# microsoft/ptgnn

Measured on NVIDIA H100. Metric: edges/sec per GNN layer, higher is better.
Workload: dtype f32

## Files before the change

ptgnn_b200/csrc/fused_mp.cu:

```cuda
#include "fused_mp.cuh"

#include <cuda_bf16.h>
#include <cuda_fp16.h>
#include <float.h>
#include <stdlib.h>

#include <type_traits>

#include "tc_common.cuh"

namespace ptgnn {
namespace fused {

using tc::mbar_arrive;
using tc::mbar_init;
using tc::mbar_wait;

constexpr int NUM_THREADS = 16 * 32;
constexpr int GATHER_WARP0 = 8, GATHER_THREADS = 64;
constexpr int SCHED_WARP = 10;
constexpr int REDUCER_WARP0 = 12;
constexpr int SCHED_READER_WARPS = 8 + 2 + 4;
constexpr int NUM_SLOTS = 3, LOOKAHEAD = 2;
constexpr int SLOT_BYTES = 32768;
constexpr int RING_BYTES = NUM_SLOTS * SLOT_BYTES;
constexpr int META_RING = 8;
constexpr int SCHED_RING = 4;
constexpr int PRODUCER_REGS = 56, CONSUMER_REGS = 184, REDUCER_REGS = 88;
static_assert(PRODUCER_REGS + 2 * CONSUMER_REGS + REDUCER_REGS <= 4 * 128, "register budgets exceed the launch allocation");
constexpr int NMAX = 64;
constexpr int ACC_PITCH = NMAX + 4;
constexpr int ACC_BYTES = kD * ACC_PITCH * 4;
constexpr int RED_BAR_ID = 1;

struct Meta {
    int32_t tloff[128];
    uint32_t endmask[4];
    int32_t n, pad[3];
};
struct Sched {
    int32_t blk, pad[3];
    int32_t off[PTGNN_MAX_EDGE_TYPES + 4];
};
constexpr int ACC_OFF = RING_BYTES;
constexpr int AGG_OFF = RING_BYTES + ACC_BYTES;
__host__ __device__ constexpr int agg_bytes(int B) { return B * kD * 4; }
constexpr int SMEM_TAIL = META_RING * (int)sizeof(Meta) + SCHED_RING * (int)sizeof(Sched) + 256 ;
constexpr int smem_bytes(int B) { return 1024 + RING_BYTES + ACC_BYTES + agg_bytes(B) + SMEM_TAIL; }
static_assert(smem_bytes(kMaxBlockTargets) <= 232448, "shared memory budget");

struct Params {
    const unsigned char *src_rows, *tgt_rows;
    const uint4 *wpack;
    const int32_t *group_off, *src_f;
    const uint8_t *tl_f;
    const int32_t *row_ptr;
    void *out;
    int num_nodes, num_blocks, B, T, reduce, out_mode;
    int32_t *status;
    unsigned long long *trace;
    Epilogue epi;
    EgcEpilogue egc;
};
constexpr int EPI_AGG = 0, EPI_EGC = 1;

__device__ __forceinline__ uint4 ldg_nc_u4(const uint4 *p) {
    uint4 r;
    asm volatile("ld.global.nc.L1::no_allocate.v4.u32 {%0,%1,%2,%3}, [%4];" : "=r"(r.x), "=r"(r.y), "=r"(r.z), "=r"(r.w) : "l"(p));
    return r;
}
__device__ __forceinline__ void named_bar_sync(int id, int threads) { asm volatile("bar.sync %0, %1;" ::"r"(id), "r"(threads) : "memory"); }
__device__ __forceinline__ uint32_t swz(int row, int q) { return (uint32_t)(row * 128 + ((q ^ (row & 7)) << 4)); }

constexpr int TRACE_ROLES = 4, TRACE_CAP = 8192;
__shared__ uint32_t trace_n[TRACE_ROLES];
__device__ __forceinline__ void trace_mark(const Params &p, int tag, uint32_t step) {
    if (p.trace == nullptr || blockIdx.x != 0) return;
    const int tid = (int)threadIdx.x;
    const int role = tid == GATHER_WARP0 * 32 ? 0 : (tid == 0 ? 1 : (tid == 128 ? 2 : (tid == REDUCER_WARP0 * 32 ? 3 : -1)));
    if (role < 0) return;
    const uint32_t n = trace_n[role];
    if (n >= TRACE_CAP) return;
    p.trace[role * TRACE_CAP + n] = ((unsigned long long)clock64() << 24) | ((unsigned long long)(step & 0xFFFFu) << 8) | (unsigned)(tag & 0xFF);
    trace_n[role] = n + 1;
}

struct Step { int blk, t, e, n, seg; };
template <int NSEG>
struct StepGen {
    const Sched *sched;
    uint64_t *sfull, *sempty;
    int T, nmax, lane;
    uint32_t it = 0;
    const Sched *tab = nullptr;
    int blk = -1, t = 0, e = 0, e1 = 0, seg = 0;
    __device__ __forceinline__ int next(Step &s) {
        for (;;) {
            if (tab == nullptr) {
                const uint32_t r = it % SCHED_RING;
                mbar_wait(&sfull[r], (it / SCHED_RING) & 1);
                blk = sched[r].blk;
                if (blk < 0) return 2;
                tab = &sched[r];
                t = -1; e = e1 = 0; seg = 0;
            }
            if (e < e1) {
                s.blk = blk; s.t = t; s.e = e; s.n = min(nmax, e1 - e); s.seg = seg;
                if (++seg == NSEG) { seg = 0; e += nmax; }
                return 0;
            }
            ++t;
            while (t < T && tab->off[t + 1] == tab->off[t]) ++t;
            if (t >= T) {
                tab = nullptr;
                s.blk = blk;
                __syncwarp();
                if (lane == 0) mbar_arrive(&sempty[it % SCHED_RING]);
                ++it;
                return 1;
            }
            e = tab->off[t]; e1 = tab->off[t + 1]; seg = 0;
        }
    }
};

template <int RED>
__device__ __forceinline__ void continue_segment(float &t, float prev, float v, uint32_t start_bit) {
    if (RED == PTGNN_REDUCE_MAX)
        asm("{\n\t.reg .pred pc;\n\tsetp.eq.u32 pc, %3, 0;\n\t@pc max.f32 %0, %1, %2;\n\t}" : "+f"(t) : "f"(prev), "f"(v), "r"(start_bit));
    else if (RED == PTGNN_REDUCE_MIN)
        asm("{\n\t.reg .pred pc;\n\tsetp.eq.u32 pc, %3, 0;\n\t@pc min.f32 %0, %1, %2;\n\t}" : "+f"(t) : "f"(prev), "f"(v), "r"(start_bit));
    else
        asm("{\n\t.reg .pred pc;\n\tsetp.eq.u32 pc, %3, 0;\n\t@pc add.f32 %0, %1, %2;\n\t}" : "+f"(t) : "f"(prev), "f"(v), "r"(start_bit));
}
__device__ __forceinline__ void sts_f32_if(uint32_t addr, float v, uint32_t bit) {
    asm volatile("{\n\t.reg .pred pe;\n\tsetp.ne.u32 pe, %2, 0;\n\t@pe st.shared.f32 [%0], %1;\n\t}" ::"r"(addr), "f"(v), "r"(bit) : "memory");
}
__device__ __forceinline__ float4 lds_f32x4(uint32_t addr) {
    float4 v;
    asm volatile("ld.shared.v4.f32 {%0, %1, %2, %3}, [%4];" : "=f"(v.x), "=f"(v.y), "=f"(v.z), "=f"(v.w) : "r"(addr));
    return v;
}
__device__ __forceinline__ void sts_f32x4(uint32_t addr, float4 v) {
    asm volatile("st.shared.v4.f32 [%0], {%1, %2, %3, %4};" ::"r"(addr), "f"(v.x), "f"(v.y), "f"(v.z), "f"(v.w) : "memory");
}
__device__ __forceinline__ float lds_f32(uint32_t addr) {
    float v;
    asm volatile("ld.shared.f32 %0, [%1];" : "=f"(v) : "r"(addr) : "memory");
    return v;
}

__device__ __forceinline__ uint32_t pack_h2(__half a, __half b) {
    return (uint32_t)__half_as_ushort(a) | ((uint32_t)__half_as_ushort(b) << 16);
}
__device__ __forceinline__ bool split_f16(float x, __half &hi, __half &lo) {
    hi = __float2half_rn(x);
    lo = __float2half_rn((x - __half2float(hi)) * 2048.0f);
    return fabsf(x) < 65504.0f;
}

template <int RED> __device__ __forceinline__ float red_identity() {
    return RED == PTGNN_REDUCE_MAX ? -FLT_MAX : (RED == PTGNN_REDUCE_MIN ? FLT_MAX : 0.0f);
}
template <int RED> __device__ __forceinline__ float red_op(float a, float m) {
    if (RED == PTGNN_REDUCE_MAX) return fmaxf(a, m);
    if (RED == PTGNN_REDUCE_MIN) return fminf(a, m);
    return a + m;
}

template <int RED>
__device__ __forceinline__ void write_out_block(const Params *p, uint32_t agg_saddr, int row0, int r_first, int r_step, int q) {
    const float IDENT = red_identity<RED>();
    const int my_hi = min(p->B, p->num_nodes - row0);
    const float4 ident4 = make_float4(IDENT, IDENT, IDENT, IDENT);
    auto finish_row = [&](auto mode_tag, auto plain_tag, int r, float4 a) {
        constexpr int MODE = decltype(mode_tag)::value;
        constexpr bool PLAIN = decltype(plain_tag)::value;
        const int v = row0 + r;
        if (!PLAIN) {
            if (RED == PTGNN_REDUCE_MEAN) {
                const int cnt = __ldg(p->row_ptr + v + 1) - __ldg(p->row_ptr + v);
                const float c = (float)(cnt < 1 ? 1 : cnt);
                a.x /= c; a.y /= c; a.z /= c; a.w /= c;
            }
            if (RED == PTGNN_REDUCE_MAX || RED == PTGNN_REDUCE_MIN) {
                if (a.x == IDENT) a.x = 0.0f;
                if (a.y == IDENT) a.y = 0.0f;
                if (a.z == IDENT) a.z = 0.0f;
                if (a.w == IDENT) a.w = 0.0f;
            }
            if (p->epi.act != PTGNN_ACT_NONE) {
                a.x = apply_act(a.x, p->epi.act); a.y = apply_act(a.y, p->epi.act);
                a.z = apply_act(a.z, p->epi.act); a.w = apply_act(a.w, p->epi.act);
            }
            if (p->epi.ln_w != nullptr) {
                float sum = (a.x + a.y) + (a.z + a.w);
#pragma unroll
                for (int o = 16; o > 0; o >>= 1) sum += __shfl_xor_sync(0xffffffffu, sum, o);
                const float mean = sum / (float)kD;
                const float dx = a.x - mean, dy = a.y - mean, dz = a.z - mean, dw = a.w - mean;
                float qq = (dx * dx + dy * dy) + (dz * dz + dw * dw);
#pragma unroll
                for (int o = 16; o > 0; o >>= 1) qq += __shfl_xor_sync(0xffffffffu, qq, o);
                const float rstd = rsqrtf(qq / (float)kD + p->epi.ln_eps);
                const float4 w = *reinterpret_cast<const float4 *>(p->epi.ln_w + q * 4);
                const float4 b = *reinterpret_cast<const float4 *>(p->epi.ln_b + q * 4);
                a.x = dx * rstd * w.x + b.x; a.y = dy * rstd * w.y + b.y;
                a.z = dz * rstd * w.z + b.z; a.w = dw * rstd * w.w + b.w;
            }
        }
        if (MODE == 1) {
            __nv_bfloat162 lo = __floats2bfloat162_rn(a.x, a.y), hi = __floats2bfloat162_rn(a.z, a.w);
            uint2 pk;
            pk.x = *reinterpret_cast<uint32_t *>(&lo); pk.y = *reinterpret_cast<uint32_t *>(&hi);
            reinterpret_cast<uint2 *>(p->out)[(size_t)v * (kD / 4) + q] = pk;
        } else if (MODE == 2) {
            const __half2 h01 = __floats2half2_rn(a.x, a.y), h23 = __floats2half2_rn(a.z, a.w);
            const float2 f01 = __half22float2(h01), f23 = __half22float2(h23);
            const __half2 l01 = __floats2half2_rn((a.x - f01.x) * 2048.0f, (a.y - f01.y) * 2048.0f);
            const __half2 l23 = __floats2half2_rn((a.z - f23.x) * 2048.0f, (a.w - f23.y) * 2048.0f);
            uint2 *row = reinterpret_cast<uint2 *>(p->out) + (size_t)v * (2 * kD / 4);
            row[q] = make_uint2(*reinterpret_cast<const uint32_t *>(&h01), *reinterpret_cast<const uint32_t *>(&h23));
            row[kD / 4 + q] = make_uint2(*reinterpret_cast<const uint32_t *>(&l01), *reinterpret_cast<const uint32_t *>(&l23));
            const float big = fmaxf(fmaxf(fabsf(a.x), fabsf(a.y)), fmaxf(fabsf(a.z), fabsf(a.w)));
            if (!(big < 65504.0f) && p->status != nullptr) *reinterpret_cast<volatile int32_t *>(p->status) = 1;
        } else {
            reinterpret_cast<float4 *>(p->out)[(size_t)v * (kD / 4) + q] = a;
        }
    };
    auto write_rows = [&](auto mode_tag, auto plain_tag) {
        for (int r0 = r_first; r0 < my_hi; r0 += 2 * r_step) {
            float4 v4[2];
#pragma unroll
            for (int u = 0; u < 2; ++u) {
                const int r = r0 + r_step * u;
                if (r < my_hi) {
                    const uint32_t rowa = agg_saddr + (uint32_t)(r * kD + q * 4) * 4u;
                    v4[u] = lds_f32x4(rowa);
                    sts_f32x4(rowa, ident4);
                }
            }
#pragma unroll
            for (int u = 0; u < 2; ++u)
                if (r0 + r_step * u < my_hi) finish_row(mode_tag, plain_tag, r0 + r_step * u, v4[u]);
        }
    };
    const bool plain = RED == PTGNN_REDUCE_SUM && p->epi.act == PTGNN_ACT_NONE && p->epi.ln_w == nullptr;
    using std::integral_constant;
    if (p->out_mode == 2) { if (plain) write_rows(integral_constant<int, 2>{}, integral_constant<bool, true>{}); else write_rows(integral_constant<int, 2>{}, integral_constant<bool, false>{}); }
    else if (p->out_mode == 1) { if (plain) write_rows(integral_constant<int, 1>{}, integral_constant<bool, true>{}); else write_rows(integral_constant<int, 1>{}, integral_constant<bool, false>{}); }
    else { if (plain) write_rows(integral_constant<int, 0>{}, integral_constant<bool, true>{}); else write_rows(integral_constant<int, 0>{}, integral_constant<bool, false>{}); }
}

__device__ __forceinline__ float bf16r(float x) { return __bfloat162float(__float2bfloat16_rn(x)); }

template <int RED>
__device__ __forceinline__ void write_out_block_egc(const Params *p, uint32_t agg_saddr, int row0, int r_first, int r_step, int q) {
    const float IDENT = red_identity<RED>();
    const int my_hi = min(p->B, p->num_nodes - row0);
    const float4 ident4 = make_float4(IDENT, IDENT, IDENT, IDENT);
    const EgcEpilogue &e = p->egc;
    const bool bf = p->out_mode == 1;
    for (int r = r_first; r < my_hi; r += r_step) {
        const uint32_t rowa = agg_saddr + (uint32_t)(r * kD + q * 4) * 4u;
        const float4 a4 = lds_f32x4(rowa);
        sts_f32x4(rowa, ident4);
        const int v = row0 + r;
        float x[4] = {a4.x, a4.y, a4.z, a4.w};
        float cdiv = 1.0f;
        if (RED == PTGNN_REDUCE_MEAN) {
            const int cnt = __ldg(p->row_ptr + v + 1) - __ldg(p->row_ptr + v);
            cdiv = (float)(cnt < 1 ? 1 : cnt);
        }
#pragma unroll
        for (int i = 0; i < 4; ++i) {
            if (RED == PTGNN_REDUCE_MEAN) x[i] /= cdiv;
            if ((RED == PTGNN_REDUCE_MAX || RED == PTGNN_REDUCE_MIN) && x[i] == IDENT) x[i] = 0.0f;
            if (bf) x[i] = bf16r(x[i]);
        }
        const float *crow = e.coef + (size_t)v * e.coef_stride;
        auto prod = [&](float A, float w) { const float t = __fmul_rn(A, w); return bf ? bf16r(t) : t; };
        const size_t orow = (size_t)v * e.out_stride;
        auto store1 = [&](int o, float s) {
            if (bf) reinterpret_cast<__nv_bfloat16 *>(p->out)[orow + o] = __float2bfloat16_rn(s);
            else reinterpret_cast<float *>(p->out)[orow + o] = s;
        };
        if (e.bases == 4 || e.bases == 8) {
            const int o = e.col0 + (e.bases == 4 ? q : q >> 1);
            const int b0 = e.bases == 4 ? 0 : 4 * (q & 1);
            const float4 w = *reinterpret_cast<const float4 *>(crow + (o / e.dh) * e.bases + b0);
            const float p0 = prod(x[0], w.x), p1 = prod(x[1], w.y), p2 = prod(x[2], w.z), p3 = prod(x[3], w.w);
            float s = __fadd_rn(__fadd_rn(__fadd_rn(p0, p1), p2), p3);
            if (e.bases == 8) {
                const float lower = __shfl_xor_sync(0xffffffffu, s, 1);
                s = __fadd_rn(__fadd_rn(__fadd_rn(__fadd_rn(lower, p0), p1), p2), p3);
                if ((q & 1) == 0) continue;
            }
            store1(o, s);
        } else if (e.bases == 2) {
            const int o = e.col0 + 2 * q;
            const float2 w0 = *reinterpret_cast<const float2 *>(crow + (o / e.dh) * 2);
            const float2 w1 = *reinterpret_cast<const float2 *>(crow + ((o + 1) / e.dh) * 2);
            const float s0 = __fadd_rn(prod(x[0], w0.x), prod(x[1], w0.y));
            const float s1 = __fadd_rn(prod(x[2], w1.x), prod(x[3], w1.y));
            if (bf) *reinterpret_cast<__nv_bfloat162 *>(reinterpret_cast<__nv_bfloat16 *>(p->out) + orow + o) = __floats2bfloat162_rn(s0, s1);
            else *reinterpret_cast<float2 *>(reinterpret_cast<float *>(p->out) + orow + o) = make_float2(s0, s1);
        } else {
            const int o = e.col0 + 4 * q;
            float s[4];
#pragma unroll
            for (int i = 0; i < 4; ++i) s[i] = prod(x[i], __ldg(crow + (o + i) / e.dh));
            if (bf) {
                __nv_bfloat162 lo = __floats2bfloat162_rn(s[0], s[1]), hi = __floats2bfloat162_rn(s[2], s[3]);
                uint2 pk;
                pk.x = *reinterpret_cast<uint32_t *>(&lo); pk.y = *reinterpret_cast<uint32_t *>(&hi);
                *reinterpret_cast<uint2 *>(reinterpret_cast<__nv_bfloat16 *>(p->out) + orow + o) = pk;
            } else {
                *reinterpret_cast<float4 *>(reinterpret_cast<float *>(p->out) + orow + o) = make_float4(s[0], s[1], s[2], s[3]);
            }
        }
    }
}

template <int NPROD, int K, int NSEG, int RED, int EPI>
__global__ void __launch_bounds__(NUM_THREADS, 1) fused_aggregate_kernel(const __grid_constant__ Params p) {
    constexpr int NPART = NPROD == 3 ? 2 : 1;
    constexpr int ROW_BYTES = K * 2 * NPART;
    constexpr int KCH = K / 64;
    constexpr int NT = NPART * KCH;
    constexpr int TILE_BYTES = NMAX * 128;
    static_assert(NT * TILE_BYTES <= SLOT_BYTES, "slot size");
    constexpr bool BF16 = NPROD == 1;

    extern __shared__ unsigned char smem_raw[];
    unsigned char *ring = smem_raw + ((1024u - (smem_u32(smem_raw) & 1023u)) & 1023u);
    float *acc_s = reinterpret_cast<float *>(ring + ACC_OFF);
    float *agg_s = reinterpret_cast<float *>(ring + AGG_OFF);
    unsigned char *tail = ring + AGG_OFF + agg_bytes(p.B);
    Meta *meta_ring = reinterpret_cast<Meta *>(tail);
    Sched *sched = reinterpret_cast<Sched *>(tail + META_RING * sizeof(Meta));
    uint64_t *bars = reinterpret_cast<uint64_t *>(tail + META_RING * sizeof(Meta) + SCHED_RING * sizeof(Sched));
    uint64_t *x_full = bars, *x_empty = bars + 3, *sched_full = bars + 6, *sched_empty = bars + 10;
    uint64_t *acc_full = bars + 14, *acc_empty = bars + 15;

    const int warp = __shfl_sync(0xffffffffu, (int)(threadIdx.x >> 5), 0);
    const int lane = threadIdx.x & 31;
    if (threadIdx.x == 0) {
        for (int s = 0; s < NUM_SLOTS; ++s) { mbar_init(&x_full[s], 2 * GATHER_THREADS); mbar_init(&x_empty[s], 8); }
        for (int r = 0; r < SCHED_RING; ++r) { mbar_init(&sched_full[r], 1); mbar_init(&sched_empty[r], SCHED_READER_WARPS); }
        mbar_init(acc_full, 8);
        mbar_init(acc_empty, 4);
        for (int r = 0; r < TRACE_ROLES; ++r) trace_n[r] = 0;
        tc::mbar_init_fence();
    }
    __syncthreads();
    const int T = p.T;

    if (warp >= REDUCER_WARP0) {
        tc::reg_dealloc<REDUCER_REGS>();
        const int d = (int)threadIdx.x - REDUCER_WARP0 * 32, rw = warp - REDUCER_WARP0;
        const uint32_t aggcol_s = smem_u32(agg_s + d);
        const uint32_t accrow_s = smem_u32(acc_s + d * ACC_PITCH);
        const float IDENT = red_identity<RED>();
        for (int r = 0; r < p.B; ++r) agg_s[r * kD + d] = IDENT;
        StepGen<NSEG> gen{sched, sched_full, sched_empty, T, NMAX, lane};
        uint32_t sg = 0;
        float acc = IDENT;
        Step s;
        for (int ev; (ev = gen.next(s)) != 2;) {
            if (ev == 1) {
                trace_mark(p, 33, sg);
                named_bar_sync(RED_BAR_ID, 128);
                if constexpr (EPI == EPI_EGC) write_out_block_egc<RED>(&p, smem_u32(agg_s), s.blk * p.B, rw, 4, lane);
                else write_out_block<RED>(&p, smem_u32(agg_s), s.blk * p.B, rw, 4, lane);
                named_bar_sync(RED_BAR_ID, 128);
                trace_mark(p, 34, sg);
                continue;
            }
            if (s.seg != NSEG - 1) continue;
            trace_mark(p, 30, sg);
            mbar_wait(acc_full, sg & 1);
            trace_mark(p, 31, sg);
            const Meta *m = &meta_ring[sg % META_RING];
            const int n = s.n;
            constexpr int W = 16;
            for (int c0 = 0; c0 < n; c0 += W) {
                uint32_t vm[W];
#pragma unroll
                for (int j = 0; j < W / 4; ++j) {
                    const float4 v4 = lds_f32x4(accrow_s + (uint32_t)(c0 + 4 * j) * 4u);
                    vm[4 * j] = __float_as_uint(v4.x); vm[4 * j + 1] = __float_as_uint(v4.y);
                    vm[4 * j + 2] = __float_as_uint(v4.z); vm[4 * j + 3] = __float_as_uint(v4.w);
                }
                uint32_t addr[W];
#pragma unroll
                for (int j = 0; j < W / 4; ++j) {
                    const int4 o = *reinterpret_cast<const int4 *>(&m->tloff[c0 + 4 * j]);
                    addr[4 * j] = aggcol_s + o.x; addr[4 * j + 1] = aggcol_s + o.y;
                    addr[4 * j + 2] = aggcol_s + o.z; addr[4 * j + 3] = aggcol_s + o.w;
                }
                const uint32_t endw = (m->endmask[c0 >> 5] >> (c0 & 31)) & 0xFFFFu;
                const uint32_t prev_end = c0 == 0 ? 1u : (m->endmask[(c0 - 1) >> 5] >> ((c0 - 1) & 31)) & 1u;
                const uint32_t startw = (endw << 1) | prev_end;
                float pre[W];
#pragma unroll
                for (int c = 0; c < W; ++c) pre[c] = lds_f32(addr[c]);
                float t[W];
                constexpr bool ADD = RED == PTGNN_REDUCE_SUM || RED == PTGNN_REDUCE_MEAN;
#pragma unroll
                for (int c = 0; c < W; ++c) {
                    const float v = __uint_as_float(vm[c]);
                    t[c] = ADD ? __fadd_rn(pre[c], v) : red_op<RED>(pre[c], v);
                }
                continue_segment<RED>(t[0], acc, __uint_as_float(vm[0]), startw & 1u);
#pragma unroll
                for (int c = 1; c < W; ++c) continue_segment<RED>(t[c], t[c - 1], __uint_as_float(vm[c]), startw & (1u << c));
                acc = t[W - 1];
#pragma unroll
                for (int c = 0; c < W; ++c) sts_f32_if(addr[c], t[c], endw & (1u << c));
            }
            __syncwarp();
            if (lane == 0) mbar_arrive(acc_empty);
            trace_mark(p, 32, sg);
            ++sg;
        }
    } else if (warp >= GATHER_WARP0) {
        tc::reg_dealloc<PRODUCER_REGS>();
        if (warp == SCHED_WARP) {
            for (uint32_t i = 0;; ++i) {
                const uint32_t r = i % SCHED_RING;
                mbar_wait(&sched_empty[r], ((i / SCHED_RING) & 1) ^ 1);
                const long long blk = (long long)blockIdx.x + (long long)i * gridDim.x;
                const bool valid = blk < p.num_blocks;
                Sched *e = &sched[r];
                if (valid) {
                    for (int t = lane; t <= T; t += 32) e->off[t] = __ldg(p.group_off + blk * T + t);
                }
                if (lane == 0) e->blk = valid ? (int)blk : -1;
                __syncwarp();
                if (lane == 0) mbar_arrive(&sched_full[r]);
                if (!valid) break;
            }
        } else if (warp < GATHER_WARP0 + GATHER_THREADS / 32) {
            const int g = (int)threadIdx.x - GATHER_WARP0 * 32;
            const int q = g & 7, rsub = g >> 3;
            StepGen<NSEG> gen{sched, sched_full, sched_empty, T, NMAX, lane};
            uint32_t c_issue = 0, c_done = 0, sgc = 0;
            Step cur, nxt;
            bool has_nxt = false;
            int idx_nxt[NMAX / 8];
            int tl_a[NMAX / 64], tl_b[NMAX / 64];
            auto fetch = [&]() {
                int ev;
                do { ev = gen.next(nxt); } while (ev == 1);
                has_nxt = ev == 0;
                if (!has_nxt) return;
                if (nxt.seg == 0) {
#pragma unroll
                    for (int i = 0; i < NMAX / 8; ++i) {
                        const int r = rsub + 8 * i;
                        idx_nxt[i] = r < nxt.n ? __ldg(p.src_f + nxt.e + r) : -1;
                    }
#pragma unroll
                    for (int half = 0; half < NMAX / 64; ++half) {
                        const int c = g + 64 * half;
                        tl_a[half] = c < nxt.n ? (int)__ldg(p.tl_f + nxt.e + c) : -1;
                        tl_b[half] = c + 1 < nxt.n ? (int)__ldg(p.tl_f + nxt.e + c + 1) : -2;
                    }
                } else {
#pragma unroll
                    for (int i = 0; i < NMAX / 8; ++i) {
                        const int r = rsub + 8 * i;
                        idx_nxt[i] = r < nxt.n ? nxt.blk * p.B + (int)__ldg(p.tl_f + nxt.e + r) : -1;
                    }
                }
            };
            auto finish_meta = [&](const Step &st) {
                if (st.seg != 0) return;
                Meta *m = &meta_ring[sgc % META_RING];
#pragma unroll
                for (int half = 0; half < NMAX / 64; ++half) {
                    const int c = g + 64 * half;
                    const bool valid = tl_a[half] >= 0;
                    const bool end = valid && tl_b[half] != tl_a[half];
                    m->tloff[c] = valid ? tl_a[half] * (kD * 4) : 0;
                    const uint32_t word = __ballot_sync(0xffffffffu, end);
                    if (lane == 0) m->endmask[c >> 5] = word;
                }
                if (g == 0) m->n = st.n;
                ++sgc;
            };
            auto issue_next = [&]() {
                cur = nxt;
                int idx[NMAX / 8];
#pragma unroll
                for (int i = 0; i < NMAX / 8; ++i) idx[i] = idx_nxt[i];
                finish_meta(cur);
                const uint32_t slot = c_issue % NUM_SLOTS;
                trace_mark(p, 1, c_issue);
                mbar_wait(&x_empty[slot], ((c_issue / NUM_SLOTS) & 1) ^ 1);
                trace_mark(p, 2, c_issue);
                const unsigned char *rows = cur.seg == 0 ? p.src_rows : p.tgt_rows;
                const uint32_t sbase = smem_u32(ring + slot * SLOT_BYTES) + swz(rsub, q);
#pragma unroll
                for (int i = 0; i < NMAX / 8; ++i) {
                    if (idx[i] >= 0) {
                        const unsigned char *src = rows + (size_t)idx[i] * ROW_BYTES + q * 16;
#pragma unroll
                        for (int ti = 0; ti < NT; ++ti)
                            cp_async16(sbase + ti * TILE_BYTES + i * 1024, src + (ti / KCH) * (K * 2) + (ti % KCH) * 128, 16);
                    }
                }
                trace_mark(p, 3, c_issue);
                ++c_issue;
            };
            fetch();
            bool more = has_nxt;
            while (more) {
                const uint32_t slot = c_issue % NUM_SLOTS;
                issue_next();
                asm volatile("cp.async.mbarrier.arrive.noinc.shared::cta.b64 [%0];" ::"r"(smem_u32(&x_full[slot])) : "memory");
                trace_mark(p, 4, c_done);
                mbar_arrive(&x_full[slot]);
                ++c_done;
                fetch();
                more = has_nxt;
            }
            cp_async_wait<0>();
        }
    } else {
        tc::reg_alloc<CONSUMER_REGS>();
        const int eg = warp >> 2, ew = warp & 3;
        const int gq = lane >> 2, tq = lane & 3;
        const int f0 = 64 * eg + 16 * ew + gq;
        StepGen<NSEG> gen{sched, sched_full, sched_empty, T, NMAX, lane};
        uint32_t sg = 0, xs = 0;
        int w_t = -1, w_seg = -1;
        uint32_t wf[NPART][K / 16][4];
        float acc_m[32], acc_c[32];
        auto load_weights = [&](const Step &st) {
            const uint32_t *wp = reinterpret_cast<const uint32_t *>(p.wpack + (size_t)(st.t * NSEG + st.seg) * NPART * (K / 8) * 128);
#pragma unroll
            for (int part = 0; part < NPART; ++part)
#pragma unroll
                for (int ks = 0; ks < K / 16; ++ks)
#pragma unroll
                    for (int i = 0; i < 4; ++i) {
                        const int c4 = (part * (K / 8) + 2 * ks + (i >> 1)), f = f0 + 8 * (i & 1);
                        wf[part][ks][i] = __ldg(wp + ((size_t)c4 * 128 + f) * 4 + tq);
                    }
            w_t = st.t; w_seg = st.seg;
            trace_mark(p, 11, xs);
        };
        auto mma = [&](auto nb_tag, uint32_t slot_addr) {
            constexpr int NB = decltype(nb_tag)::value;
#pragma unroll
            for (int ks = 0; ks < K / 16; ++ks) {
                const int kc = ks >> 2, kk = ks & 3;
                const uint64_t x_hi = tc::make_smem_desc_sw128(slot_addr + kc * TILE_BYTES) + kk * 2;
                const uint64_t x_lo = tc::make_smem_desc_sw128(slot_addr + (KCH + kc) * TILE_BYTES) + kk * 2;
                auto one = [&](float (&dacc)[32], const uint32_t (&a)[4], uint64_t desc) {
                    if (NB == 1) tc::wgmma_16_rs_n16<BF16>(dacc, a, desc);
                    else if (NB == 2) tc::wgmma_16_rs_n32<BF16>(dacc, a, desc);
                    else if (NB == 3) tc::wgmma_16_rs_n48<BF16>(dacc, a, desc);
                    else tc::wgmma_16_rs_n64<BF16>(dacc, a, desc);
                };
                one(acc_m, wf[0][ks], x_hi);
                if (NPROD == 3) {
                    one(acc_c, wf[0][ks], x_lo);
                    one(acc_c, wf[NPART - 1][ks], x_hi);
                }
            }
        };
        Step s, nx;
        int ev = gen.next(s);
        while (ev != 2) {
            if (ev == 0) {
                trace_mark(p, 10, xs);
                if (s.t != w_t || s.seg != w_seg) load_weights(s);
                const uint32_t slot = xs % NUM_SLOTS;
                mbar_wait(&x_full[slot], (xs / NUM_SLOTS) & 1);
                tc::fence_proxy_async_smem();
                trace_mark(p, 12, xs);
                if (tc::warp_uniform(s.seg) == 0) {
#pragma unroll
                    for (int i = 0; i < 32; ++i) { acc_m[i] = 0.0f; acc_c[i] = 0.0f; }
                }
                const uint32_t slot_addr = smem_u32(ring + slot * SLOT_BYTES);
                const int nb = tc::warp_uniform((s.n + 15) >> 4);
                tc::wgmma_fence();
                using std::integral_constant;
                if (nb == 1) mma(integral_constant<int, 1>{}, slot_addr);
                else if (nb == 2) mma(integral_constant<int, 2>{}, slot_addr);
                else if (nb == 3) mma(integral_constant<int, 3>{}, slot_addr);
                else mma(integral_constant<int, 4>{}, slot_addr);
                tc::wgmma_commit();
                trace_mark(p, 13, xs);
                tc::wgmma_wait<0>();
                tc::fence_acc(acc_m);
                if (NPROD == 3) tc::fence_acc(acc_c);
                __syncwarp();
                if (lane == 0) mbar_arrive(&x_empty[slot]);
                trace_mark(p, 14, xs);
                ++xs;
                const int evn = gen.next(nx);
                if (evn == 0 && (nx.t != w_t || nx.seg != w_seg)) load_weights(nx);
                if (s.seg == NSEG - 1) {
                    trace_mark(p, 20, sg);
                    mbar_wait(acc_empty, (sg & 1) ^ 1);
                    trace_mark(p, 21, sg);
#pragma unroll
                    for (int j = 0; j < 8; ++j) {
                        if (8 * j < 16 * nb) {
#pragma unroll
                        for (int h = 0; h < 2; ++h) {
                            float v0 = acc_m[4 * j + 2 * h], v1 = acc_m[4 * j + 2 * h + 1];
                            if (NPROD == 3) {
                                v0 = fmaf(acc_c[4 * j + 2 * h], 1.0f / 2048.0f, v0); v1 = fmaf(acc_c[4 * j + 2 * h + 1], 1.0f / 2048.0f, v1);
                            } else {
                                v0 = __bfloat162float(__float2bfloat16_rn(v0)); v1 = __bfloat162float(__float2bfloat16_rn(v1));
                            }
                            *reinterpret_cast<float2 *>(acc_s + (f0 + 8 * h) * ACC_PITCH + 8 * j + 2 * tq) = make_float2(v0, v1);
                        }
                        }
                    }
                    __syncwarp();
                    if (lane == 0) mbar_arrive(acc_full);
                    trace_mark(p, 22, sg);
                    ++sg;
                }
                s = nx; ev = evn;
                continue;
            }
            ev = gen.next(s);
        }
    }
}

__global__ void __launch_bounds__(256) pack_states_kernel(const float *__restrict__ h, long long rows, int K,
                                                          uint4 *__restrict__ out, int32_t *__restrict__ status) {
    const long long total = rows * (K / 8);
    bool bad = false;
    for (long long i = (long long)blockIdx.x * blockDim.x + threadIdx.x; i < total; i += (long long)gridDim.x * blockDim.x) {
        const long long row = i / (K / 8);
        const int c8 = (int)(i - row * (K / 8));
        const float4 a = ld_stream_f4(reinterpret_cast<const float4 *>(h + row * K + c8 * 8));
        const float4 b = ld_stream_f4(reinterpret_cast<const float4 *>(h + row * K + c8 * 8 + 4));
        const float x[8] = {a.x, a.y, a.z, a.w, b.x, b.y, b.z, b.w};
        __half hi[8], lo[8];
#pragma unroll
        for (int j = 0; j < 8; ++j) bad |= !split_f16(x[j], hi[j], lo[j]);
        uint4 vh, vl;
        vh.x = pack_h2(hi[0], hi[1]); vh.y = pack_h2(hi[2], hi[3]); vh.z = pack_h2(hi[4], hi[5]); vh.w = pack_h2(hi[6], hi[7]);
        vl.x = pack_h2(lo[0], lo[1]); vl.y = pack_h2(lo[2], lo[3]); vl.z = pack_h2(lo[4], lo[5]); vl.w = pack_h2(lo[6], lo[7]);
        uint4 *dst = out + row * (K / 4);
        dst[c8] = vh;
        dst[K / 8 + c8] = vl;
    }
    if (bad && status != nullptr) *reinterpret_cast<volatile int32_t *>(status) = 1;
}

struct WeightSrc {
    const float *w[PTGNN_MAX_EDGE_TYPES];
};
template <int NPROD>
__global__ void __launch_bounds__(256) pack_weights_kernel(const __grid_constant__ WeightSrc src, int num_types, int K, int nseg,
                                                           RowMap rows, uint4 *__restrict__ out, int32_t *__restrict__ status) {
    constexpr int NPART = NPROD == 3 ? 2 : 1;
    const int per_mat = nseg * (K / 8) * 128;
    const long long total = (long long)num_types * per_mat;
    bool bad = false;
    for (long long i = (long long)blockIdx.x * blockDim.x + threadIdx.x; i < total; i += (long long)gridDim.x * blockDim.x) {
        const int t = (int)(i / per_mat);
        int r = (int)(i - (long long)t * per_mat);
        const int seg = r / ((K / 8) * 128);
        r -= seg * (K / 8) * 128;
        const int c4 = r / 128, d = r % 128;
        int srow = d;
        if (rows.bases > 0) {
            const int o = rows.col0 + d / rows.bases, b = d % rows.bases;
            srow = ((o / rows.dh) * rows.bases + b) * rows.dh + o % rows.dh;
        }
        const float *row = src.w[t] + (size_t)srow * (nseg * K) + seg * K + c4 * 8;
        float x[8];
#pragma unroll
        for (int j = 0; j < 8; ++j) x[j] = row[j];
        const size_t base = ((size_t)(t * nseg + seg) * NPART) * (K / 8) * 128;
        if (NPROD == 3) {
            __half hi[8], lo[8];
#pragma unroll
            for (int j = 0; j < 8; ++j) bad |= !split_f16(x[j], hi[j], lo[j]);
            uint4 vh, vl;
            vh.x = pack_h2(hi[0], hi[1]); vh.y = pack_h2(hi[2], hi[3]); vh.z = pack_h2(hi[4], hi[5]); vh.w = pack_h2(hi[6], hi[7]);
            vl.x = pack_h2(lo[0], lo[1]); vl.y = pack_h2(lo[2], lo[3]); vl.z = pack_h2(lo[4], lo[5]); vl.w = pack_h2(lo[6], lo[7]);
            out[base + (size_t)c4 * 128 + d] = vh;
            out[base + (size_t)(K / 8 + c4) * 128 + d] = vl;
        } else {
            uint4 v;
            __nv_bfloat162 p0 = __floats2bfloat162_rn(x[0], x[1]), p1 = __floats2bfloat162_rn(x[2], x[3]);
            __nv_bfloat162 p2 = __floats2bfloat162_rn(x[4], x[5]), p3 = __floats2bfloat162_rn(x[6], x[7]);
            v.x = *reinterpret_cast<uint32_t *>(&p0); v.y = *reinterpret_cast<uint32_t *>(&p1);
            v.z = *reinterpret_cast<uint32_t *>(&p2); v.w = *reinterpret_cast<uint32_t *>(&p3);
            out[base + (size_t)c4 * 128 + d] = v;
        }
    }
    if (bad && status != nullptr) *reinterpret_cast<volatile int32_t *>(status + 1) = 1;
}

bool supported(int nprod, int K, int D, int use_target) {
    (void)use_target;
    if (D != kD) return false;
    if (nprod == 3) return K == 64 || K == 128;
    if (nprod == 1) return K == 64 || K == 128 || K == 256;
    return false;
}
size_t packed_weight_bytes(int nprod, int num_types, int K, int use_target) {
    const int nseg = use_target ? 2 : 1, npart = nprod == 3 ? 2 : 1;
    return ws_slice((size_t)num_types * nseg * npart * (K / 8) * 128, 16);
}
size_t packed_state_bytes(int nprod, int64_t rows, int K) {
    return nprod == 3 ? ws_slice((size_t)rows * K * 4 + 16, 1) : 0;
}
int recommended_block_targets(int64_t num_nodes) {
    if (num_nodes <= 0) return kMaxBlockTargets;
    const int64_t waves = ceil_div(num_nodes, (int64_t)kMaxBlockTargets * 132);
    int64_t B = ceil_div(num_nodes, waves * 132);
    B = (B + 7) / 8 * 8;
    if (B < 8) B = 8;
    if (B > kMaxBlockTargets) B = kMaxBlockTargets;
    return (int)B;
}

int pack_weights(int nprod, int num_types, int K, int use_target, const float *const *weights, void *packed, int32_t *status,
                 cudaStream_t st, RowMap rows) {
    WeightSrc src{};
    for (int t = 0; t < num_types; ++t) src.w[t] = weights[t];
    const int nseg = use_target ? 2 : 1;
    {
        TimedScope timed__(PTGNN_KERNEL_PACK, st);
        if (nprod == 3) pack_weights_kernel<3><<<132, 256, 0, st>>>(src, num_types, K, nseg, rows, static_cast<uint4 *>(packed), status);
        else pack_weights_kernel<1><<<132, 256, 0, st>>>(src, num_types, K, nseg, rows, static_cast<uint4 *>(packed), status);
    }
    PTGNN_LAUNCHED();
    return PTGNN_OK;
}

int pack_states(const float *h, int64_t rows, int K, void *packed, int32_t *status, cudaStream_t st) {
    if (rows <= 0) return PTGNN_OK;
    const int64_t items = rows * (K / 8);
    const unsigned grid = (unsigned)(ceil_div(items, 256) < 132 * 8 ? ceil_div(items, 256) : 132 * 8);
    {
        TimedScope timed__(PTGNN_KERNEL_PACK, st);
        pack_states_kernel<<<grid, 256, 0, st>>>(h, (long long)rows, K, static_cast<uint4 *>(packed), status);
    }
    PTGNN_LAUNCHED();
    return PTGNN_OK;
}

template <int NPROD, int K, int NSEG, int RED, int EPI = EPI_AGG>
static int launch_one(const Params &p, cudaStream_t st) {
    auto kernel = fused_aggregate_kernel<NPROD, K, NSEG, RED, EPI>;
    const int smem = smem_bytes(p.B);
    PTGNN_CUDA(cudaFuncSetAttribute(kernel, cudaFuncAttributeMaxDynamicSharedMemorySize, smem));
    const int sms = sm_count();
    const int grid = p.num_blocks < sms ? p.num_blocks : sms;
    {
        TimedScope timed__(PTGNN_KERNEL_MESSAGE, st);
        kernel<<<grid, NUM_THREADS, smem, st>>>(p);
    }
    PTGNN_LAUNCHED();
    return PTGNN_OK;
}
template <int NPROD, int K, int NSEG, int EPI = EPI_AGG>
static int launch_red(const Params &p, cudaStream_t st) {
    switch (p.reduce) {
        case PTGNN_REDUCE_SUM: return launch_one<NPROD, K, NSEG, PTGNN_REDUCE_SUM, EPI>(p, st);
        case PTGNN_REDUCE_MEAN: return launch_one<NPROD, K, NSEG, PTGNN_REDUCE_MEAN, EPI>(p, st);
        case PTGNN_REDUCE_MAX: return launch_one<NPROD, K, NSEG, PTGNN_REDUCE_MAX, EPI>(p, st);
        default: return launch_one<NPROD, K, NSEG, PTGNN_REDUCE_MIN, EPI>(p, st);
    }
}
template <int NPROD, int K>
static int launch_seg(const Params &p, int use_target, bool egc, cudaStream_t st) {
    if (egc) return launch_red<NPROD, K, 1, EPI_EGC>(p, st);
    return use_target ? launch_red<NPROD, K, 2>(p, st) : launch_red<NPROD, K, 1>(p, st);
}

static unsigned long long *g_trace_dev = nullptr;
static unsigned long long *trace_buffer() {
    static int want = -1;
    if (want < 0) { const char *e = getenv("PTGNN_FUSED_TRACE"); want = (e && e[0] == '1') ? 1 : 0; }
    if (!want) return nullptr;
    if (!g_trace_dev && cudaMalloc(&g_trace_dev, TRACE_ROLES * TRACE_CAP * 8) != cudaSuccess) return nullptr;
    cudaMemset(g_trace_dev, 0, TRACE_ROLES * TRACE_CAP * 8);
    return g_trace_dev;
}

int aggregate(const AggregateArgs &a, cudaStream_t st) {
    PTGNN_CHECK_ARG(supported(a.nprod, a.K, kD, a.use_target), "fused aggregate: unsupported nprod=%d K=%d", a.nprod, a.K);
    PTGNN_CHECK_ARG(a.block_targets >= 8 && a.block_targets <= kMaxBlockTargets, "fused aggregate: block_targets=%d out of [8, %d]",
                    a.block_targets, kMaxBlockTargets);
    PTGNN_CHECK_ARG(a.num_types > 0 && a.num_types <= PTGNN_MAX_EDGE_TYPES, "fused aggregate: bad num_types=%d", a.num_types);
    PTGNN_CHECK_ARG(a.reduce >= PTGNN_REDUCE_SUM && a.reduce <= PTGNN_REDUCE_MIN, "fused aggregate: bad reduce %d", a.reduce);
    if (a.num_nodes <= 0) return PTGNN_OK;
    PTGNN_CHECK_ARG(a.src_rows && a.group_off && a.packed_weights && a.out, "fused aggregate: null pointer");
    PTGNN_CHECK_ARG(!a.use_target || a.tgt_rows, "fused aggregate: null target rows");
    PTGNN_CHECK_ARG(a.reduce != PTGNN_REDUCE_MEAN || a.row_ptr, "fused aggregate: mean needs row_ptr");
    Params p{};
    p.src_rows = static_cast<const unsigned char *>(a.src_rows);
    p.tgt_rows = static_cast<const unsigned char *>(a.tgt_rows);
    p.wpack = static_cast<const uint4 *>(a.packed_weights);
    p.group_off = a.group_off; p.src_f = a.src_f; p.tl_f = a.tl_f; p.row_ptr = a.row_ptr;
    p.out = a.out; p.num_nodes = (int)a.num_nodes; p.B = a.block_targets;
    p.num_blocks = (int)ceil_div(a.num_nodes, a.block_targets);
    p.T = a.num_types; p.reduce = a.reduce; p.out_mode = a.out_mode; p.status = a.status; p.epi = a.epi;
    p.trace = trace_buffer();
    const bool egc = a.egc != nullptr;
    if (egc) {
        const EgcEpilogue &e = *a.egc;
        PTGNN_CHECK_ARG(!a.use_target && (a.out_mode == 0 || a.out_mode == 1), "fused aggregate: the EGC write-out takes one segment, fp32 / bf16 output");
        PTGNN_CHECK_ARG((e.bases == 1 || e.bases == 2 || e.bases == 4 || e.bases == 8) && e.dh > 0 && e.coef && e.col0 >= 0 &&
                            e.col0 + kD / e.bases <= e.out_stride && e.coef_stride % 4 == 0,
                        "fused aggregate: bad EGC write-out (bases %d, dh %d, col0 %d, stride %d)", e.bases, e.dh, e.col0, e.out_stride);
        p.egc = e;
    }
#ifdef PTGNN_FUSED_QUICK
    return a.nprod == 3 ? launch_one<3, 128, 1, PTGNN_REDUCE_SUM>(p, st) : launch_one<1, 128, 1, PTGNN_REDUCE_SUM>(p, st);
#else
    if (a.nprod == 3) {
        if (a.K == 64) return launch_seg<3, 64>(p, a.use_target, egc, st);
        return launch_seg<3, 128>(p, a.use_target, egc, st);
    }
    if (a.K == 64) return launch_seg<1, 64>(p, a.use_target, egc, st);
    if (a.K == 128) return launch_seg<1, 128>(p, a.use_target, egc, st);
    return launch_seg<1, 256>(p, a.use_target, egc, st);
#endif
}

}
}

extern "C" int ptgnn_b200_debug_fused_trace(unsigned long long *out) {
    using namespace ptgnn::fused;
    if (!g_trace_dev) return 0;
    if (out != nullptr) {
        cudaDeviceSynchronize();
        cudaMemcpy(out, g_trace_dev, TRACE_ROLES * TRACE_CAP * 8, cudaMemcpyDeviceToHost);
    }
    return TRACE_CAP;
}
```

Measured before the change: 1.338 billion.

## Pack weights in per-lane fragment order and alternate consumer warpgroups via named barriers

Weights are now packed in the exact register-fragment order each lane needs, so one 16-byte load per k-step replaces four scattered 4-byte loads when reloading weights. Separately, the two consumer warpgroups take turns issuing their WGMMA batches through a ping-pong pair of named barriers, so their tensor-core issue no longer collides and one group's epilogue can overlap the other's math. The turn-taking adds barrier waits, and the arrive/sync pairing at loop exit has to stay balanced to avoid deadlock or leftover barrier state.

```diff
diff --git a/ptgnn_b200/csrc/fused_mp.cu b/ptgnn_b200/csrc/fused_mp.cu
--- a/ptgnn_b200/csrc/fused_mp.cu
+++ b/ptgnn_b200/csrc/fused_mp.cu
@@ -32,6 +32,7 @@
 constexpr int ACC_PITCH = NMAX + 4;
 constexpr int ACC_BYTES = kD * ACC_PITCH * 4;
 constexpr int RED_BAR_ID = 1;
+constexpr int TURN_BAR = 2;
 
 struct Meta {
     int32_t tloff[128];
@@ -70,6 +71,7 @@
     return r;
 }
 __device__ __forceinline__ void named_bar_sync(int id, int threads) { asm volatile("bar.sync %0, %1;" ::"r"(id), "r"(threads) : "memory"); }
+__device__ __forceinline__ void named_bar_arrive(int id, int threads) { asm volatile("bar.arrive %0, %1;" ::"r"(id), "r"(threads) : "memory"); }
 __device__ __forceinline__ uint32_t swz(int row, int q) { return (uint32_t)(row * 128 + ((q ^ (row & 7)) << 4)); }
 
 constexpr int TRACE_ROLES = 4, TRACE_CAP = 8192;
@@ -539,16 +541,14 @@
         uint32_t wf[NPART][K / 16][4];
         float acc_m[32], acc_c[32];
         auto load_weights = [&](const Step &st) {
-            const uint32_t *wp = reinterpret_cast<const uint32_t *>(p.wpack + (size_t)(st.t * NSEG + st.seg) * NPART * (K / 8) * 128);
+            const uint4 *wp = p.wpack + (size_t)(st.t * NSEG + st.seg) * NPART * (K / 16) * 256 + (4 * eg + ew) * 32 + lane;
 #pragma unroll
             for (int part = 0; part < NPART; ++part)
 #pragma unroll
-                for (int ks = 0; ks < K / 16; ++ks)
-#pragma unroll
-                    for (int i = 0; i < 4; ++i) {
-                        const int c4 = (part * (K / 8) + 2 * ks + (i >> 1)), f = f0 + 8 * (i & 1);
-                        wf[part][ks][i] = __ldg(wp + ((size_t)c4 * 128 + f) * 4 + tq);
-                    }
+                for (int ks = 0; ks < K / 16; ++ks) {
+                    const uint4 v = __ldg(wp + (part * (K / 16) + ks) * 256);
+                    wf[part][ks][0] = v.x; wf[part][ks][1] = v.y; wf[part][ks][2] = v.z; wf[part][ks][3] = v.w;
+                }
             w_t = st.t; w_seg = st.seg;
             trace_mark(p, 11, xs);
         };
@@ -573,7 +573,9 @@
             }
         };
         Step s, nx;
+        if (eg == 1) named_bar_arrive(TURN_BAR, 256);
         int ev = gen.next(s);
+        if (ev == 2 && eg == 0) named_bar_sync(TURN_BAR, 256);
         while (ev != 2) {
             if (ev == 0) {
                 trace_mark(p, 10, xs);
@@ -588,6 +590,8 @@
                 }
                 const uint32_t slot_addr = smem_u32(ring + slot * SLOT_BYTES);
                 const int nb = tc::warp_uniform((s.n + 15) >> 4);
+                named_bar_sync(TURN_BAR + eg, 256);
+                trace_mark(p, 15, xs);
                 tc::wgmma_fence();
                 using std::integral_constant;
                 if (nb == 1) mma(integral_constant<int, 1>{}, slot_addr);
@@ -595,6 +599,7 @@
                 else if (nb == 3) mma(integral_constant<int, 3>{}, slot_addr);
                 else mma(integral_constant<int, 4>{}, slot_addr);
                 tc::wgmma_commit();
+                named_bar_arrive(TURN_BAR + (eg ^ 1), 256);
                 trace_mark(p, 13, xs);
                 tc::wgmma_wait<0>();
                 tc::fence_acc(acc_m);
@@ -633,6 +638,7 @@
                 continue;
             }
             ev = gen.next(s);
+            if (ev == 2 && eg == 0) named_bar_sync(TURN_BAR, 256);
         }
     }
 }
@@ -667,25 +673,28 @@
 __global__ void __launch_bounds__(256) pack_weights_kernel(const __grid_constant__ WeightSrc src, int num_types, int K, int nseg,
                                                            RowMap rows, uint4 *__restrict__ out, int32_t *__restrict__ status) {
     constexpr int NPART = NPROD == 3 ? 2 : 1;
-    const int per_mat = nseg * (K / 8) * 128;
+    const int per_mat = nseg * (K / 16) * 256;
     const long long total = (long long)num_types * per_mat;
     bool bad = false;
     for (long long i = (long long)blockIdx.x * blockDim.x + threadIdx.x; i < total; i += (long long)gridDim.x * blockDim.x) {
         const int t = (int)(i / per_mat);
         int r = (int)(i - (long long)t * per_mat);
-        const int seg = r / ((K / 8) * 128);
-        r -= seg * (K / 8) * 128;
-        const int c4 = r / 128, d = r % 128;
-        int srow = d;
-        if (rows.bases > 0) {
-            const int o = rows.col0 + d / rows.bases, b = d % rows.bases;
-            srow = ((o / rows.dh) * rows.bases + b) * rows.dh + o % rows.dh;
-        }
-        const float *row = src.w[t] + (size_t)srow * (nseg * K) + seg * K + c4 * 8;
+        const int seg = r / ((K / 16) * 256);
+        r -= seg * (K / 16) * 256;
+        const int ks = r / 256, rb = (r % 256) / 32, ln = r % 32;
         float x[8];
 #pragma unroll
-        for (int j = 0; j < 8; ++j) x[j] = row[j];
-        const size_t base = ((size_t)(t * nseg + seg) * NPART) * (K / 8) * 128;
+        for (int j = 0; j < 4; ++j) {
+            const int d = 16 * rb + (ln >> 2) + 8 * (j & 1), k = 16 * ks + 2 * (ln & 3) + 8 * (j >> 1);
+            int srow = d;
+            if (rows.bases > 0) {
+                const int o = rows.col0 + d / rows.bases, b = d % rows.bases;
+                srow = ((o / rows.dh) * rows.bases + b) * rows.dh + o % rows.dh;
+            }
+            const float *row = src.w[t] + (size_t)srow * (nseg * K) + seg * K + k;
+            x[2 * j] = row[0]; x[2 * j + 1] = row[1];
+        }
+        const size_t base = ((size_t)(t * nseg + seg) * NPART) * (K / 16) * 256 + (size_t)ks * 256 + r % 256;
         if (NPROD == 3) {
             __half hi[8], lo[8];
 #pragma unroll
@@ -693,15 +702,15 @@
             uint4 vh, vl;
             vh.x = pack_h2(hi[0], hi[1]); vh.y = pack_h2(hi[2], hi[3]); vh.z = pack_h2(hi[4], hi[5]); vh.w = pack_h2(hi[6], hi[7]);
             vl.x = pack_h2(lo[0], lo[1]); vl.y = pack_h2(lo[2], lo[3]); vl.z = pack_h2(lo[4], lo[5]); vl.w = pack_h2(lo[6], lo[7]);
-            out[base + (size_t)c4 * 128 + d] = vh;
-            out[base + (size_t)(K / 8 + c4) * 128 + d] = vl;
+            out[base] = vh;
+            out[base + (size_t)(K / 16) * 256] = vl;
         } else {
             uint4 v;
             __nv_bfloat162 p0 = __floats2bfloat162_rn(x[0], x[1]), p1 = __floats2bfloat162_rn(x[2], x[3]);
             __nv_bfloat162 p2 = __floats2bfloat162_rn(x[4], x[5]), p3 = __floats2bfloat162_rn(x[6], x[7]);
             v.x = *reinterpret_cast<uint32_t *>(&p0); v.y = *reinterpret_cast<uint32_t *>(&p1);
             v.z = *reinterpret_cast<uint32_t *>(&p2); v.w = *reinterpret_cast<uint32_t *>(&p3);
-            out[base + (size_t)c4 * 128 + d] = v;
+            out[base] = v;
         }
     }
     if (bad && status != nullptr) *reinterpret_cast<volatile int32_t *>(status + 1) = 1;
```

Result: faster. 1.378 billion (median of 6 runs) (+3.0%).
